# hungdinhxuan/real-time-deepfake-speech-detection

Hardware: AMD Instinct MI355X
Metric: utterances/sec (4 s @ 16 kHz) (higher is better)
Workload: dtype fp16

## Files before the change

real-time-deepfake-speech-detection_amd/csrc/afx_conformer.hip:

```cpp
#include "afx_common.h"
#include "afx_kernels.h"

namespace afx {

__global__ void conf_tokens_kernel(const float* __restrict__ ll, const float* __restrict__ cls, float bn_scale,
                                   float bn_shift, int T, int E, float* __restrict__ out, int raw) {
  const int b = blockIdx.y;
  const long n = (long)(T + 1) * E;
  for (long i = (long)blockIdx.x * blockDim.x + threadIdx.x; i < n; i += (long)gridDim.x * blockDim.x) {
    const int row = (int)(i / E), c = (int)(i % E);
    float v;
    if (row == 0)
      v = cls[c];
    else if (raw)
      v = ll[((long)b * T + row - 1) * E + c];
    else
      v = selu(fmaf(ll[((long)b * T + row - 1) * E + c], bn_scale, bn_shift));
    out[(long)b * n + i] = v;
  }
}
const char* launch_conf_tokens(const float* ll, const float* cls, float bn_scale, float bn_shift, int B, int T,
                               int E, float* out, hipStream_t s, bool raw) {
  hipLaunchKernelGGL(conf_tokens_kernel, dim3(16, B), dim3(256), 0, s, ll, cls, bn_scale, bn_shift, T, E, out, raw ? 1 : 0);
  hipError_t e = hipGetLastError();
  return e == hipSuccess ? nullptr : hipGetErrorString(e);
}

template <int DH, class HT, bool REL>
__global__ __launch_bounds__(256) void conf_attn_kernel(const float* __restrict__ q, long ldq,
                                                        const float* __restrict__ kv, long ldkv,
                                                        const float* __restrict__ rel, int max_pos, int N, int H,
                                                        int KB, typename HT::T* __restrict__ out, long ldo,
                                                        const int* __restrict__ lens, int len_add) {
  typedef typename HT::T Tt;
  extern __shared__ __attribute__((aligned(16))) float sm_f[];
  const int Nrow = N;
  if (lens) N = lens[blockIdx.y] + len_add;

  const int i0 = blockIdx.z * 256;
  const int nq = min(256, N - i0);
  float* Ks = sm_f;
  float* Vs = Ks + (long)KB * DH;
  float* Es = Vs + (long)KB * DH;
  const int h = blockIdx.x, b = blockIdx.y, tid = threadIdx.x;
  const int inner = H * DH;
  const bool live = tid < nq;
  const int i = i0 + (live ? tid : nq - 1);
  const float scale = 1.0f / sqrtf((float)DH);
  float qv[DH], o[DH];
  const float* qrow = q + ((long)b * Nrow + i) * ldq + h * DH;
#pragma unroll
  for (int d = 0; d < DH; d += 4) {
    const f32x4 t = *(const f32x4*)(qrow + d);
    qv[d] = t[0] * scale; qv[d + 1] = t[1] * scale; qv[d + 2] = t[2] * scale; qv[d + 3] = t[3] * scale;
    o[d] = o[d + 1] = o[d + 2] = o[d + 3] = 0.f;
  }
  float m = -1e30f, l = 0.f;
  for (int jb = 0; jb < N; jb += KB) {
    const int nk = min(KB, N - jb);
    if (jb) __syncthreads();
    for (int idx = tid; idx < nk * (DH / 4); idx += 256) {
// ... 60 lines not shown
  Tt* orow = out + ((long)b * Nrow + i) * ldo + h * DH;
#pragma unroll
  for (int d = 0; d < DH; d += 4) {
    typename HT::V4 v4;
    v4[0] = (Tt)(o[d] * rl); v4[1] = (Tt)(o[d + 1] * rl); v4[2] = (Tt)(o[d + 2] * rl); v4[3] = (Tt)(o[d + 3] * rl);
    *(typename HT::V4*)(orow + d) = v4;
  }
}

static int g_conf_attn_block = 0;
void conf_attn_set_block(int v) { g_conf_attn_block = v > 0 ? (v + 3) & ~3 : 0; }

template <int DH, class HT, bool REL>
static hipError_t launch_conf_attn_t(const float* q, long ldq, const float* kv, long ldkv, const float* rel,
                                     int max_pos, int B, int N, int H, void* out, long ldo, hipStream_t s,
                                     const int* lens, int len_add) {
  auto lds_of = [&](int kb) { return (int)((2L * kb + (REL ? min(256, N) + kb - 1 : 0)) * DH * sizeof(float)); };
  int KB = N;
  if (g_conf_attn_block && g_conf_attn_block < N) KB = g_conf_attn_block;
  else if (N > 256 || lds_of(N) > 160 * 1024) KB = 64;
  const int lds = lds_of(KB);
  static LdsLimit lim;
  if (hipError_t e = lim.ensure((const void*)conf_attn_kernel<DH, HT, REL>, lds); e != hipSuccess) return e;
  hipLaunchKernelGGL((conf_attn_kernel<DH, HT, REL>), dim3(H, B, (N + 255) / 256), dim3(256), lds, s, q, ldq, kv, ldkv, rel,
                     max_pos, N, H, KB, (typename HT::T*)out, ldo, lens, len_add);
  return hipGetLastError();
}

const char* launch_conf_attn(const float* q, long ldq, const float* kv, long ldkv, const float* rel, int max_pos,
                             int B, int N, int H, int dh, void* out_h, long ldo, int dtype, hipStream_t s,
                             const int* lens, int len_add) {
  if (N <= 0 || B <= 0 || B > 65535) return "conf_attn: bad shape";
  if ((ldq % 4) || (ldkv % 4) || (ldo % 4)) return "conf_attn: row strides must be multiples of 4";
  hipError_t e = hipSuccess;
#define AFX_CA(DHv)                                                                                             \
  AFX_DISPATCH_HT(dtype, e = launch_conf_attn_t<DHv, HT, true>(q, ldq, kv, ldkv, rel, max_pos, B, N, H, out_h, ldo, s, lens, len_add))
  if (!rel) {
    if (dh != 64 || dtype != DT_FP32) return "conf_attn: the no-relative-term form is the fp32 trunk attention (dh 64)";
    e = launch_conf_attn_t<64, F32T, false>(q, ldq, kv, ldkv, nullptr, 0, B, N, H, out_h, ldo, s, lens, len_add);
  }
  else if (dh == 36) { AFX_CA(36); }
  else if (dh == 32) { AFX_CA(32); }
  else if (dh == 64) { AFX_CA(64); }
  else return "conf_attn: supported head dims are 32, 36 (emb 144 / 4 heads) and 64";
#undef AFX_CA
  return e == hipSuccess ? nullptr : hipGetErrorString(e);
}

constexpr int CA_KEYS = 224, CA_VT_STRIDE = 232, CA_RS = 228, CA_NKT = 14, CA_KS = 7;

template <class HT, int DH, int NW>
__global__ __launch_bounds__(64 * NW) void conf_attn_mfma_kernel(const float* __restrict__ q, long ldq,
                                                             const float* __restrict__ kv, long ldkv,
                                                             const typename HT::T* __restrict__ rel_h, int max_pos,
                                                             int N, int H, typename HT::T* __restrict__ out, long ldo,
                                                             const int* __restrict__ lens, int len_add) {
  typedef typename HT::T Tt;
  typedef typename HT::V8 V8;
  typedef typename HT::V4 V4;
  const int Nrow = N;
  if (lens) N = lens[blockIdx.y] + len_add;
  constexpr int DT = (DH + 15) / 16;
  static_assert(DH % 4 == 0 && DH <= 64, "head dim");
  extern __shared__ __attribute__((aligned(16))) float sm_f[];
  char* sm = (char*)sm_f;
  char* k_lds = sm;
  Tt* vt_lds = (Tt*)(sm + CA_KEYS * 128);
  float* r_lds = (float*)(sm + CA_KEYS * 128 + 16 * DT * CA_VT_STRIDE * 2);
  constexpr int NT = 64 * NW;

  const int h = blockIdx.x, b = blockIdx.y;
// ... 22 lines not shown
        V4 kh;
#pragma unroll
        for (int i = 0; i < 4; ++i) kh[i] = (Tt)kreg[it][i];
        const int c = q4 >> 1;
        *(V4*)(k_lds + key * 128 + ((c ^ ((key >> 1) & 7)) * 16) + (q4 & 1) * 8) = kh;
#pragma unroll
        for (int i = 0; i < 4; ++i) vt_lds[(q4 * 4 + i) * CA_VT_STRIDE + key] = (Tt)vreg[it][i];
      }
    }
  }
  __syncthreads();

  const int ql = lane & 15, g = lane >> 4;
  const float scale = 1.0f / sqrtf((float)DH);
  float* rw = r_lds + wave * 16 * CA_RS;
  const int nqt = (N + 15) >> 4;
  for (int qt = wave; qt < nqt; qt += NW) {
    const int q0 = qt * 16;
    int qrow = q0 + ql;
    qrow = qrow < N ? qrow : N - 1;
    V8 qf[2];
    {
      const float* qp = q + ((long)b * Nrow + qrow) * ldq + h * DH;
#pragma unroll
      for (int ks = 0; ks < 2; ++ks)
#pragma unroll
        for (int half = 0; half < 2; ++half) {
          const int d = ks * 32 + g * 8 + half * 4;
          f32x4 t = f32x4{0.f, 0.f, 0.f, 0.f};
          if (d < DH) t = *(const f32x4*)(qp + d);
#pragma unroll
// ... 118 lines not shown
        const int d = nt * 16 + g * 4;
        if (d < DH) {
          V4 hv;
#pragma unroll
          for (int c = 0; c < 4; ++c) hv[c] = (Tt)(o[nt][c] * rinv);
          *(V4*)(out + ((long)b * Nrow + qi) * ldo + h * DH + d) = hv;
        }
      }
    }
  }
}

template <int DH, int NW>
__global__ __launch_bounds__(64 * NW) void conf_attn_split_kernel(const float* __restrict__ q, long ldq, const float* __restrict__ kv, long ldkv,
                                                                  const float* __restrict__ rel64, int max_pos, int N, int H,
                                                                  float* __restrict__ out, long ldo, const int* __restrict__ lens, int len_add) {
  typedef _Float16 Tt;
  typedef f16x8 V8;
  typedef f16x4 V4;
  const int Nrow = N;
  if (lens) N = lens[blockIdx.y] + len_add;
  constexpr int DT = (DH + 15) / 16;
  static_assert(DH % 4 == 0 && DH <= 64, "head dim");
  extern __shared__ __attribute__((aligned(16))) float sm_f[];
  char* sm = (char*)sm_f;
  constexpr int KB = CA_KEYS * 128, VB = 16 * DT * CA_VT_STRIDE * 2;
  char* k_lds[2] = {sm, sm + KB};
  Tt* vt_lds[2] = {(Tt*)(sm + 2 * KB), (Tt*)(sm + 2 * KB + VB)};
  float* r_lds = (float*)(sm + 2 * KB + 2 * VB);
  constexpr int NT = 64 * NW;
  const int h = blockIdx.x, b = blockIdx.y;
// ... 43 lines not shown
        *(V4*)(k_lds[0] + off) = kh;
        *(V4*)(k_lds[1] + off) = kl;
#pragma unroll
        for (int i = 0; i < 4; ++i) {
          vt_lds[0][(q4 * 4 + i) * CA_VT_STRIDE + key] = vh[i];
          vt_lds[1][(q4 * 4 + i) * CA_VT_STRIDE + key] = vl[i];
        }
      }
    }
  }
  __syncthreads();

  const int ql = lane & 15, g = lane >> 4;
  const float scale = 1.0f / sqrtf((float)DH);
  float* rw = r_lds + wave * 16 * CA_RS;
  const int nqt = (N + 15) >> 4;
  for (int qt = wave; qt < nqt; qt += NW) {
    const int q0 = qt * 16;
    int qrow = q0 + ql;
    qrow = qrow < N ? qrow : N - 1;
    V8 qh[2], qlo[2];
    {
      const float* qp = q + ((long)b * Nrow + qrow) * ldq + h * DH;
#pragma unroll
      for (int ks = 0; ks < 2; ++ks) {
        f32x4 t[2];
#pragma unroll
        for (int half = 0; half < 2; ++half) {
          const int d = ks * 32 + g * 8 + half * 4;
          t[half] = f32x4{0.f, 0.f, 0.f, 0.f};
          if (d < DH) t[half] = *(const f32x4*)(qp + d);
// ... 129 lines not shown
#pragma unroll
      for (int nt = 0; nt < DT; ++nt) {
        const int d = nt * 16 + g * 4;
        if (d < DH) *(f32x4*)(out + ((long)b * Nrow + qi) * ldo + h * DH + d) = o[nt] * rinv;
      }
#ifdef SHAW_DBG
      if (g == 0) {
        out[((long)b * Nrow + qi) * ldo + h * DH + 0] = mx;
        out[((long)b * Nrow + qi) * ldo + h * DH + 1] = sum;
      }
#endif
    }
  }
}
const char* launch_conf_attn_split(const float* q, long ldq, const float* kv, long ldkv, const float* rel64, int max_pos, int B, int N,
                                   int H, int dh, float* out, long ldo, hipStream_t s, const int* lens, int len_add) {
  if (dh != 36) return "conf_attn_split: built for head dim 36 (emb 144 / 4 heads)";
  if (N <= 0 || N + 15 > CA_KEYS || B <= 0 || B > 65535) return "conf_attn_split: 1..209 tokens";
  if ((ldq % 4) || (ldkv % 4) || (ldo % 4)) return "conf_attn_split: row strides must be multiples of 4";
  constexpr int DT = 3, NW = 4;
  const int lds = 2 * CA_KEYS * 128 + 2 * 16 * DT * CA_VT_STRIDE * 2 + NW * 16 * CA_RS * 4;
  static LdsLimit lim;
  hipError_t e = lim.ensure((const void*)conf_attn_split_kernel<36, NW>, lds);
  if (e == hipSuccess) {
    hipLaunchKernelGGL((conf_attn_split_kernel<36, NW>), dim3(H, B), dim3(64 * NW), lds, s, q, ldq, kv, ldkv, rel64, max_pos, N, H, out, ldo, lens, len_add);
    e = hipGetLastError();
  }
  return e == hipSuccess ? nullptr : hipGetErrorString(e);
}

constexpr int CAL_KB = 128, CAL_VT_STRIDE = 136, CAL_RS = 148, CAL_NKT = 8, CAL_KS = 4, CAL_RT = 9;

template <class HT, int DH>
__global__ __launch_bounds__(256, 2) void conf_attn_mfma_long_kernel(const float* __restrict__ q, long ldq,
                                                                  const float* __restrict__ kv, long ldkv,
                                                                  const typename HT::T* __restrict__ rel_h, int max_pos,
                                                                  int N, int H, typename HT::T* __restrict__ out, long ldo,
                                                                  const int* __restrict__ lens, int len_add) {
  typedef typename HT::T Tt;
  typedef typename HT::V8 V8;
// ... 159 lines not shown
#pragma unroll
        for (int c = 0; c < 4; ++c) hv[c] = (Tt)(o[nt][c] * rinv);
        *(V4*)(out + ((long)b * Nrow + qi) * ldo + h * DH + d) = hv;
      }
    }
  }
}

static int g_conf_attn_force_long = 0;
void conf_attn_mfma_set_force_long(int v) { g_conf_attn_force_long = v != 0; }
static int g_conf_attn_waves = 7;
void conf_attn_mfma_set_waves(int v) { g_conf_attn_waves = v == 4 ? 4 : 7; }

const char* launch_conf_attn_mfma(const float* q, long ldq, const float* kv, long ldkv, const void* rel_h, int max_pos,
                                  int B, int N, int H, int dh, void* out_h, long ldo, int dtype, hipStream_t s,
                                  const int* lens, int len_add) {
  if (dh != 36) return "conf_attn_mfma: built for head dim 36 (emb 144 / 4 heads)";
  if (N <= 0 || B <= 0 || B > 65535) return "conf_attn_mfma: bad shape";
  if (dtype == DT_FP32) return "conf_attn_mfma: half-precision operands only";
  if ((ldq % 4) || (ldkv % 4) || (ldo % 4)) return "conf_attn_mfma: row strides must be multiples of 4";
  constexpr int DT = 3;
  if (N + 15 > CA_KEYS || g_conf_attn_force_long) {
    const int ldsl = CAL_KB * 128 + 16 * DT * CAL_VT_STRIDE * 2 + 4 * 16 * CAL_RS * 4;
    hipError_t el = hipSuccess;
    static LdsLimit liml[2];
    dim3 grid(H, B, (N + 63) / 64);
    if (dtype == DT_BF16) {
      el = liml[0].ensure((const void*)conf_attn_mfma_long_kernel<BF16, 36>, ldsl);
      if (el == hipSuccess)
        hipLaunchKernelGGL((conf_attn_mfma_long_kernel<BF16, 36>), grid, dim3(256), ldsl, s, q, ldq, kv, ldkv, (const __bf16*)rel_h,
                           max_pos, N, H, (__bf16*)out_h, ldo, lens, len_add);
    } else {
      el = liml[1].ensure((const void*)conf_attn_mfma_long_kernel<FP16, 36>, ldsl);
      if (el == hipSuccess)
        hipLaunchKernelGGL((conf_attn_mfma_long_kernel<FP16, 36>), grid, dim3(256), ldsl, s, q, ldq, kv, ldkv, (const _Float16*)rel_h,
                           max_pos, N, H, (_Float16*)out_h, ldo, lens, len_add);
    }
    if (el == hipSuccess) el = hipGetLastError();
    return el == hipSuccess ? nullptr : hipGetErrorString(el);
  }
  const int nw = N > 64 && g_conf_attn_waves != 4 ? 7 : 4;
  const int lds = CA_KEYS * 128 + 16 * DT * CA_VT_STRIDE * 2 + nw * 16 * CA_RS * 4;
  hipError_t e = hipSuccess;
  static LdsLimit lim[4];
#define AFX_CAM(HTv, NWv, slot, Tv)                                                                                      \
  do {                                                                                                                   \
    e = lim[slot].ensure((const void*)conf_attn_mfma_kernel<HTv, 36, NWv>, lds);                                         \
    if (e == hipSuccess)                                                                                                 \
      hipLaunchKernelGGL((conf_attn_mfma_kernel<HTv, 36, NWv>), dim3(H, B), dim3(64 * NWv), lds, s, q, ldq, kv, ldkv,    \
                         (const Tv*)rel_h, max_pos, N, H, (Tv*)out_h, ldo, lens, len_add);                               \
  } while (0)
  if (dtype == DT_BF16) {
    if (nw == 7) AFX_CAM(BF16, 7, 0, __bf16); else AFX_CAM(BF16, 4, 1, __bf16);
  } else {
    if (nw == 7) AFX_CAM(FP16, 7, 2, _Float16); else AFX_CAM(FP16, 4, 3, _Float16);
  }
#undef AFX_CAM
  if (e == hipSuccess) e = hipGetLastError();
  return e == hipSuccess ? nullptr : hipGetErrorString(e);
}

template <class HT>
__global__ __launch_bounds__(256) void conf_dwconv_kernel(const float* __restrict__ x, long ldx,
                                                          const float* __restrict__ w, const float* __restrict__ bias,
                                                          const float* __restrict__ bn_scale,
                                                          const float* __restrict__ bn_shift, int N, int NC, int C, int k,
                                                          typename HT::T* __restrict__ out, long ldo,
                                                          const int* __restrict__ lens, int len_add) {
  typedef typename HT::T Tt;
  const int Nrow = N;
  if (lens) N = lens[blockIdx.y] + len_add;
  constexpr bool EXACT = sizeof(Tt) == 4;
  constexpr int KMAX = 31, TB = 8;
  extern __shared__ __attribute__((aligned(16))) float sm_f[];
  float* sm = sm_f;
  const int c0 = blockIdx.x * 32, b = blockIdx.y, tid = threadIdx.x;
  const int pl = k / 2;
  const int f0 = blockIdx.z * NC, nc = min(NC, N - f0);
  const int rows = nc + KMAX - 1 + TB;
  float* us = sm;
  const int cl = tid & 31, tl = tid >> 5;
  const int c = c0 + cl;
  const bool cok = c < C;
  for (int r = tl; r < rows; r += 8) {
    const int t = f0 + r - pl;
    float u = 0.f;
    if (cok && t >= 0 && t < N) {
      const float* row = x + ((long)b * Nrow + t) * ldx;
      u = row[c] * (EXACT ? sigmoid_acc(row[C + c]) : sigmoid_fast(row[C + c]));
    }
    us[r * 32 + cl] = u;
  }
  float wr[KMAX];
#pragma unroll
  for (int j = 0; j < KMAX; ++j) wr[j] = (cok && j < k) ? w[(long)c * k + j] : 0.f;
  const float bi = cok ? bias[c] : 0.f, sc = cok ? bn_scale[c] : 0.f, sh = cok ? bn_shift[c] : 0.f;
  __syncthreads();
  const int per = (nc + 7) / 8;
  const int t_end = min(nc, (tl + 1) * per);
  for (int t0 = tl * per; t0 < t_end; t0 += TB) {
    float win[TB + KMAX - 1];
#pragma unroll
// ... 5 lines not shown
    for (int j = 0; j < KMAX; ++j)
#pragma unroll
      for (int u = 0; u < TB; ++u) acc[u] = fmaf(wr[j], win[u + j], acc[u]);
    if (cok) {
#pragma unroll
      for (int u = 0; u < TB; ++u) {
        const float y = fmaf(acc[u], sc, sh);
        if (t0 + u < t_end) out[((long)b * Nrow + f0 + t0 + u) * ldo + c] = (Tt)(EXACT ? swish(y) : swish_fast(y));
      }
    }
  }
}

const char* launch_conf_dwconv(const float* x, long ldx, const float* w, const float* bias, const float* bn_scale,
                               const float* bn_shift, int B, int N, int C, int k, void* out_h, long ldo, int dtype,
                               hipStream_t s, const int* lens, int len_add) {
  if (k > 31) return "conf_dwconv: depthwise kernels up to 31 taps";
  if (N <= 0 || B <= 0 || B > 65535) return "conf_dwconv: bad shape";
  const int NC = N < 1024 ? N : 1024;
  const int lds = (NC + 31 - 1 + 8) * 32 * (int)sizeof(float);
  dim3 grid((C + 31) / 32, B, (N + NC - 1) / NC);
  hipError_t e = hipSuccess;
  static LdsLimit lim[3];
  if (dtype < 0 || dtype > 2) return "conf_dwconv: unknown dtype";
  AFX_DISPATCH_HT(dtype, {
    e = lim[dtype].ensure((const void*)conf_dwconv_kernel<HT>, lds);
    if (e == hipSuccess)
      hipLaunchKernelGGL(conf_dwconv_kernel<HT>, grid, dim3(256), lds, s, x, ldx, w, bias, bn_scale, bn_shift, N, NC, C, k,
                         (HT::T*)out_h, ldo, lens, len_add);
  });
  if (e == hipSuccess) e = hipGetLastError();
  return e == hipSuccess ? nullptr : hipGetErrorString(e);
}

__global__ void small_linear_kernel(const float* __restrict__ x, long row_stride, int rows, int K,
                                    const float* __restrict__ w, const float* __restrict__ b, int N,
                                    float* __restrict__ out, int* __restrict__ nonfinite) {
  const int lane = threadIdx.x & 63;
  const int r = blockIdx.x * (blockDim.x >> 6) + (threadIdx.x >> 6);
  if (r >= rows) return;
  const float* xr = x + (long)r * row_stride;
  for (int n = 0; n < N; ++n) {
    float a = 0.f;
    for (int kk = lane; kk < K; kk += 64) a = fmaf(xr[kk], w[(long)n * K + kk], a);
// ... 18 lines not shown
```

real-time-deepfake-speech-detection_amd/csrc/afx_conformer_fused.hip:

```cpp
#include "afx_common.h"
#include "afx_kernels.h"

#ifndef CHAIN_DBG
#define CHAIN_DBG 0
#endif

namespace afx {

namespace {

constexpr int ET = 9;
constexpr int EK = 5;
constexpr int HT6 = 6;
constexpr int RING = 4, BUFSZ = 32 * 1024, DUMP = RING * BUFSZ;
constexpr int PARAMS = DUMP + 1024;
#ifndef CHAIN_NWAVE
#define CHAIN_NWAVE 4
#endif
constexpr int NWAVE = CHAIN_NWAVE;
constexpr int DPW = 32 / NWAVE;
static_assert(NWAVE == 8 || NWAVE == 4, "wave count");
template <int N>
__device__ __forceinline__ void chain_wait_vmcnt() {
  static_assert(N >= 0 && N < 64, "vmcnt is a 6-bit counter");
// ... 299 lines not shown
    for (int j = 0; j < ET; ++j) {
      const f32x4 bb = *(const f32x4*)(prm + CP_FF_B2 + j * 16 + kq * 4);
      x[j] += 0.5f * (o[j] + bb);
    }
  }
};

}

template <class HT, int STAGE, bool S3>
__global__ __launch_bounds__(64 * NWAVE) void conf_chain_kernel(ConfChainArgs p) {
  typedef Chain<HT, STAGE, S3> C;
  typedef typename C::AF AF;
  extern __shared__ __attribute__((aligned(16))) char smem[];
  C c(p, smem);
  const long row = ((long)blockIdx.x * NWAVE + c.wave) * 16 + c.r16;
  const bool ok = row < p.M;
  const long rc = ok ? row : p.M - 1;

  f32x4 x[ET];
#pragma unroll
  for (int j = 0; j < ET; ++j) x[j] = *(const f32x4*)(p.x_in + rc * p.E + j * 16 + c.kq * 4);
  AF ain[ET];
  if constexpr (STAGE != 0) {
#pragma unroll
    for (int t = 0; t < (STAGE == 1 ? EK : ET); ++t) ain[t] = c.load_frag(p.in_h, rc, p.ld_in_h, t * 32 + c.kb);
  }
#pragma unroll
  for (int j = 0; j < ET; ++j) asm volatile("" : "+v"(x[j]));
  if constexpr (STAGE != 0) {
#pragma unroll
    for (int t = 0; t < (STAGE == 1 ? EK : ET); ++t) {
      asm volatile("" : "+v"(ain[t].h));
// ... 66 lines not shown
    c.feed_forward(x);
    f32x4 y[ET];
    c.layernorm(x, c.prm + CP_LN2_G, c.prm + CP_LN2_B, y);
    if (ok) {
#pragma unroll
      for (int j = 0; j < ET; ++j) *(f32x4*)(p.x_out + row * p.E + j * 16 + c.kq * 4) = y[j];
    }
  }
}

template <class HT, int STAGE, bool S3>
static hipError_t launch_conf_chain_t(const ConfChainArgs& p, hipStream_t s) {
  constexpr int lds = PARAMS + (kChainParamFloats + (S3 ? kChainScaleFloats : 0)) * 4;
  static LdsLimit lim;
  if (hipError_t e = lim.ensure((const void*)conf_chain_kernel<HT, STAGE, S3>, lds); e != hipSuccess) return e;
  hipLaunchKernelGGL((conf_chain_kernel<HT, STAGE, S3>), dim3((unsigned)((p.M + 16 * NWAVE - 1) / (16 * NWAVE))), dim3(64 * NWAVE), lds, s, p);
  return hipGetLastError();
}

const char* launch_conf_chain(const ConfChainArgs& p, int stage, int dtype, hipStream_t s) {
  if (p.E != 16 * ET || p.Ep < 32 * EK || p.FFp != 4 * 16 * ET) return "conf_chain: the fused Conformer chains are built for emb 144 / ff 576";
  if (dtype == DT_FP32) return "conf_chain: half-precision operands only";
  if (p.M <= 0 || stage < 0 || stage > 2) return "conf_chain: bad arguments";
  hipError_t e;
  if (dtype == DT_FP16X3)
    e = stage == 0 ? launch_conf_chain_t<FP16, 0, true>(p, s) : stage == 1 ? launch_conf_chain_t<FP16, 1, true>(p, s) : launch_conf_chain_t<FP16, 2, true>(p, s);
  else if (dtype == DT_BF16)
    e = stage == 0 ? launch_conf_chain_t<BF16, 0, false>(p, s) : stage == 1 ? launch_conf_chain_t<BF16, 1, false>(p, s) : launch_conf_chain_t<BF16, 2, false>(p, s);
  else
    e = stage == 0 ? launch_conf_chain_t<FP16, 0, false>(p, s) : stage == 1 ? launch_conf_chain_t<FP16, 1, false>(p, s) : launch_conf_chain_t<FP16, 2, false>(p, s);
  return e == hipSuccess ? nullptr : hipGetErrorString(e);
}

}
```

real-time-deepfake-speech-detection_amd/csrc/afx_engine.hip:

```cpp
#include <hip/hip_runtime.h>

#include <algorithm>
#include <cmath>
#include <cstdarg>
#include <cstdio>
#include <cstring>
#include <string>
#include <unordered_map>
#include <unordered_set>
#include <vector>

#include "../../include/afx.h"
#include "afx_common.h"
#include "afx_kernels.h"
#include "afx_aasist.h"

using namespace afx;

static thread_local char g_err[512] = "";
static int fail(const char* fmt, ...) {
  va_list ap;
  va_start(ap, fmt);
  vsnprintf(g_err, sizeof g_err, fmt, ap);
  va_end(ap);
// ... 590 lines not shown
    off += bytes;
    return p;
  }
};

struct Ws {
  int T[7];
  void *bufA = nullptr, *bufB = nullptr, *feats_h = nullptr, *xpad = nullptr, *hbuf = nullptr, *qkv = nullptr, *att = nullptr, *ff = nullptr,
       *ssl_h = nullptr;
  float *tmp32 = nullptr, *x = nullptr, *ssl_f = nullptr;
  void* s3planes = nullptr;
  size_t s3bytes = 0;
  float* gn_stats = nullptr;
  int* lens = nullptr;
  float *bucket_f = nullptr, *bucket_logits = nullptr;
  float *ll32 = nullptr, *xc = nullptr, *qkv32 = nullptr, *glu32 = nullptr;
  void *hc = nullptr, *hid = nullptr, *ao = nullptr, *u = nullptr;
  AasistWs aa;
};

static size_t carve(const afx_engine* e, int B, int L, int Tfeat, void* base, Ws* w, int T5 = 0, bool ragged = false) {
  Carver c(base);
  const size_t hs = dtype_size(e->dt);
  int T = Tfeat;
  w->lens = nullptr;
  w->bucket_f = w->bucket_logits = nullptr;
  if (L > 0 || T5 > 0) {
    if (L > 0) {
      conv_lengths(L, w->T);
      const size_t n0 = (size_t)B * w->T[0] * kC, n1 = (size_t)B * w->T[1] * kC;
// ... 462 lines not shown
    n2.out_h = w.hbuf; n2.ldo_h = kD;
    KOK(launch_rownorm(n2, dt, s));
    TAP(lp + "ln2", w.hbuf, (size_t)M * kD, true, kD);
    GemmArgs f1 = plain_gemm(w.hbuf, kD, e->w1[l], kD, M, kF, kD);
    f1.bias = e->F(P + "fc1.bias"); f1.act = ACT_GELU;
    f1.out_h = w.ff; f1.ldo_h = kF;
    KOK(launch_gemm(f1, dt, 1, s));
    TAP(lp + "ff", w.ff, (size_t)M * kF, true, kF);
    KOK(resid_product(w.ff, kF, e->w2[l], kF, e->F(P + "fc2.bias")));
    if (e->taps_on) {
      const std::string nm = "layer" + std::to_string(l);
      if (tap(e, nm.c_str(), w.x, (size_t)M * kD, false, s)) return 1;
    }
  }
  RowNormArgs nf = plain_norm(w.x, kD, M, kD, e->F("ssl.encoder.layer_norm.weight"), e->F("ssl.encoder.layer_norm.bias"));
  nf.out_f = w.ssl_f; nf.ldo_f = kD;
  nf.out_h = w.ssl_h; nf.ldo_h = kD;
  nf.nonfinite = e->nonfinite;
  KOK(launch_rownorm(nf, dt, s));
  if (tap(e, "ssl", w.ssl_f, (size_t)M * kD, false, s)) return 1;
  return 0;
}

static int run_conformer(afx_engine* e, int B, int T, Ws& w, float* logits, hipStream_t s, const float* tokens = nullptr,
                         float* embedding = nullptr) {
  const int dt = e->dt, E = e->E, Ep = e->Ep, N = T + 1, M = B * N;
  if (tokens) {
    KOK(timed(PC_MISC, 0, s, [&] { return launch_conf_tokens(tokens, e->F("conformer.class_token"), 1.f, 0.f, B, T, E, w.xc, s, true); }));
  } else {
    GemmArgs ll = plain_gemm(w.ssl_h, kD, e->conf_ll, kD, B * T, E, kD);
    ll.bias = e->F("LL.bias");
// ... 9 lines not shown
  const int chain_dt = e->s3 ? DT_FP16X3 : dt;
  HIP_OK(hipMemsetAsync(w.ao, 0, (size_t)M * Ep * hs, s));
  if (!fused) {
    HIP_OK(hipMemsetAsync(w.hc, 0, (size_t)M * Ep * hs, s));
    HIP_OK(hipMemsetAsync(w.u, 0, (size_t)M * e->C2p * hs, s));
    if (e->FFp != e->FF) HIP_OK(hipMemsetAsync(w.hid, 0, (size_t)M * e->FFp * hs, s));
  }
  for (int b = 0; fused && b < e->nblk; ++b) {
    const std::string P = "conformer.encoder_blocks." + std::to_string(b) + ".";
    ConfBlock& K = e->blk[b];
    ConfChainArgs c;
    memset(&c, 0, sizeof c);
    c.M = M; c.E = E; c.Ep = Ep; c.FFp = e->FFp;
    c.x_in = w.xc; c.x_out = w.xc;
    auto ff = [&](void* w1, void* w2) { c.ff_w1 = w1; c.ff_w2 = w2; };
    const double ff_fl = 2.0 * M * E * e->FF * 2;
    ff(K.ff1_w1, K.ff1_w2);
    c.params = K.chain_prm[0];
    c.w_a = K.wqkv; c.ld_w_a = Ep;
    c.out2 = w.qkv32; c.ld_out2 = 3 * e->inner;
    KOK(timed(PC_CONF_CHAIN, ff_fl + 2.0 * M * E * 3 * e->inner, s, [&] { return launch_conf_chain(c, 0, chain_dt, s); }));
    const std::string bp = "b" + std::to_string(b) + ".";
    TAP(bp + "xa", w.xc, (size_t)M * E, false, E);
    TAP(bp + "qkv", w.qkv32, (size_t)M * 3 * e->inner, false, 3 * e->inner);
    KOK(timed(PC_CONF_ATTN, 6.0 * B * e->heads * (double)N * N * e->dh, s, [&] {
      if (e->conf_attn_mfma && dt != DT_FP32 && e->dh == 36)
        return launch_conf_attn_mfma(w.qkv32, 3 * e->inner, w.qkv32 + e->inner, 3 * e->inner, K.rel_h, 512, B, N, e->heads,
                                     e->dh, w.ao, Ep, dt, s, w.lens, 1);
      if (e->conf_attn_mfma && e->s3 && e->dh == 36 && N <= 209)
        return launch_conf_attn_split(w.qkv32, 3 * e->inner, w.qkv32 + e->inner, 3 * e->inner, (const float*)K.rel_h, 512, B, N,
                                      e->heads, e->dh, (float*)w.ao, Ep, s, w.lens, 1);
      return launch_conf_attn(w.qkv32, 3 * e->inner, w.qkv32 + e->inner, 3 * e->inner,
                              e->F(P + "attn.fn.rel_pos_emb.weight"), 512, B, N, e->heads, e->dh, w.ao, Ep, dt, s, w.lens, 1);
    }));
    TAP(bp + "ao", w.ao, (size_t)M * Ep, true, Ep);
    c.in_h = w.ao; c.ld_in_h = Ep;
    c.params = K.chain_prm[1];
    c.w_a = K.wout;
    c.w_b = K.pw1;
    c.out2 = w.glu32; c.ld_out2 = 2 * e->C2;
    KOK(timed(PC_CONF_CHAIN, 2.0 * M * E * (e->inner + 2 * e->C2), s, [&] { return launch_conf_chain(c, 1, chain_dt, s); }));
    TAP(bp + "xb", w.xc, (size_t)M * E, false, E);
    TAP(bp + "glu", w.glu32, (size_t)M * 2 * e->C2, false, 2 * e->C2);
    KOK(timed(PC_CONF_DWCONV, 2.0 * B * N * e->C2 * e->ck, s, [&] {
      return launch_conf_dwconv(w.glu32, 2 * e->C2, e->F(P + "conv.net.4.conv.weight"),
                                e->F(P + "conv.net.4.conv.bias"), K.bn_scale, K.bn_shift, B, N, e->C2, e->ck, w.u,
                                e->C2p, dt, s, w.lens, 1);
    }));
    TAP(bp + "u", w.u, (size_t)M * e->C2p, true, e->C2p);
    c.in_h = w.u; c.ld_in_h = e->C2p;
    c.params = K.chain_prm[2];
    c.w_a = K.pw2; c.ld_w_a = e->C2p;
    ff(K.ff2_w1, K.ff2_w2);
    c.w_b = nullptr; c.out2 = nullptr;
    KOK(timed(PC_CONF_CHAIN, ff_fl + 2.0 * M * e->C2 * E, s, [&] { return launch_conf_chain(c, 2, chain_dt, s); }));
    if (e->taps_on) {
      const std::string nm = "block" + std::to_string(b);
      if (tap(e, nm.c_str(), w.xc, (size_t)M * E, false, s)) return 1;
    }
  }
  for (int b = 0; !fused && b < e->nblk; ++b) {
    const std::string P = "conformer.encoder_blocks." + std::to_string(b) + ".";
    ConfBlock& K = e->blk[b];
    const std::string bp = "b" + std::to_string(b) + ".";
    auto norm_to_h = [&](const char* nm) -> const char* {
      RowNormArgs n = plain_norm(w.xc, E, M, E, e->F(P + nm + ".weight"), e->F(P + nm + ".bias"));
      n.out_h = w.hc; n.ldo_h = Ep;
      return launch_rownorm(n, dt, s);
    };
    auto feed_forward = [&](const char* ff, void* w1, void* w2) -> int {
// ... 1101 lines not shown
    for (int k = 0; k < nb; ++k)
      HIP_OK(hipMemcpyAsync(logits + (size_t)idx[k] * 2, w.bucket_logits + (size_t)k * 2, 8, hipMemcpyDeviceToDevice, s));
  }
  return 0;
}

extern "C" int afx_ssl_forward_ragged(afx_handle h, const float* wave, int B, int Lmax, const int* n_samples, float* feats,
                                      int* n_frames, void* ws, size_t ws_bytes, void* stream) {
  if (check_call(h, wave, B, Lmax, feats, ws, true)) return 1;
  if (!n_samples) return fail("afx_ssl_forward_ragged: null lengths");
  if (h->cfg.pre_emphasis) return fail("afx_ssl_forward_ragged: engine-side pre-emphasis is not supported on ragged batches");
  if (h->cfg.extractor_mode == AFX_EXTRACTOR_GROUP_NORM) return fail("afx_ssl_forward_ragged: the group-norm extractor normalises over the whole clip; zero padding would enter its statistics");
  Ws w;
  const size_t needb = carve(h, B, Lmax, 0, ws, &w, 0, true);
  if (ws_bytes < needb) return fail("afx_ssl_forward_ragged: workspace too small (%zu < %zu bytes)", ws_bytes, needb);
  hipStream_t s = (hipStream_t)stream;
  std::vector<int> frames;
  if (ragged_setup(h, B, Lmax, n_samples, w, frames, s)) return 1;
  begin_call(h, &w);
  if (run_trunk(h, wave, B, Lmax, w, s)) return 1;
  const int Tmax = w.T[6];
  HIP_OK(hipMemcpyAsync(feats, w.ssl_f, (size_t)B * Tmax * kD * 4, hipMemcpyDeviceToDevice, s));
  for (int b = 0; b < B; ++b) {
    if (frames[b] < Tmax)
      HIP_OK(hipMemsetAsync(feats + ((size_t)b * Tmax + frames[b]) * kD, 0, (size_t)(Tmax - frames[b]) * kD * 4, s));
    if (n_frames) n_frames[b] = frames[b];
  }
  return 0;
}

extern "C" int afx_ssl_forward(afx_handle h, const float* wave, int B, int L, float* feats, void* ws, size_t ws_bytes,
                               void* stream) {
  if (check_call(h, wave, B, L, feats, ws, true)) return 1;
  Ws w;
  const size_t needb = carve(h, B, L, 0, ws, &w);
  if (ws_bytes < needb) return fail("afx_ssl_forward: workspace too small (%zu < %zu bytes)", ws_bytes, needb);
  hipStream_t s = (hipStream_t)stream;
  begin_call(h, &w);
  if (run_trunk(h, wave, B, L, w, s)) return 1;
  HIP_OK(hipMemcpyAsync(feats, w.ssl_f, (size_t)B * w.T[6] * kD * 4, hipMemcpyDeviceToDevice, s));
  return 0;
}

__global__ void f32_to_half_kernel(const float* in, uint16_t* out, size_t n, int is_bf16) {
  for (size_t i = (size_t)blockIdx.x * blockDim.x + threadIdx.x; i < n; i += (size_t)gridDim.x * blockDim.x) {
    if (is_bf16) {
      __bf16 v = (__bf16)in[i];
      memcpy(&out[i], &v, 2);
    } else {
      _Float16 v = (_Float16)in[i];
      memcpy(&out[i], &v, 2);
// ... 287 lines not shown
```

real-time-deepfake-speech-detection_amd/csrc/afx_kernels.h:

```cpp
#pragma once
#include <hip/hip_runtime.h>
#include <stdint.h>

namespace afx {

enum DType { DT_BF16 = 0, DT_FP16 = 1, DT_FP32 = 2, DT_FP16X3 = 3 };
inline size_t dtype_size(int dt) { return dt == DT_FP32 || dt == DT_FP16X3 ? 4 : 2; }
constexpr float kS3ScaleBounded = 16.f;
constexpr float kS3ScaleFree = 1.f;
__host__ __device__ inline long s3_pair_index(long k) { return ((k >> 5) << 6) + (k & 31); }

struct GemmArgs {
  const void* A;
  const void* W;
  int M, N, K;
  int k_algo;
  int rpb;
  long a_batch, a_row;
  int kchunk;
  long kchunk_stride;
  long ldw;
  long g_a, g_w;
  int g_n;
  const float* bias;
// ... 114 lines not shown
                              bool out_pairs = false, float out_scale = 1.f);
const char* launch_mhsa_ring(const void* ring, void* out, int S, int H, int q_tile, const int* cnt, int dtype, hipStream_t s);
const char* launch_mhsa_ring_split(const float* ring, float* out, int S, int H, int q_tile, const int* cnt, hipStream_t s,
                                   bool out_pairs = false, float out_scale = 1.f);
const char* launch_mhsa_ring_tab(const void* ring, void* out, int S, int H, int q_tile, const int* tab, int dtype, hipStream_t s);
const char* launch_mhsa_ring_split_tab(const float* ring, float* out, int S, int H, int q_tile, const int* tab, hipStream_t s,
                                       bool out_pairs, float out_scale);
const char* launch_mhsa_ring_active(const void* ring, void* out, int A, int H, const int* tab, int dtype, hipStream_t s);
const char* launch_mhsa_ring_split_active(const float* ring, float* out, int A, int H, const int* tab, hipStream_t s, bool out_pairs,
                                          float out_scale);

const char* launch_conf_tokens(const float* ll, const float* cls, float bn_scale, float bn_shift, int B, int T,
                               int E, float* out, hipStream_t s, bool raw = false);
const char* launch_conf_attn(const float* q, long ldq, const float* kv, long ldkv, const float* rel, int max_pos,
                             int B, int N, int H, int dh, void* out_h, long ldo, int dtype, hipStream_t s,
                             const int* lens = nullptr, int len_add = 0);
const char* launch_conf_attn_split(const float* q, long ldq, const float* kv, long ldkv, const float* rel64, int max_pos, int B, int N,
                                   int H, int dh, float* out, long ldo, hipStream_t s, const int* lens = nullptr, int len_add = 0);
const char* launch_conf_attn_mfma(const float* q, long ldq, const float* kv, long ldkv, const void* rel_h, int max_pos,
                                  int B, int N, int H, int dh, void* out_h, long ldo, int dtype, hipStream_t s,
                                  const int* lens = nullptr, int len_add = 0);
const char* launch_conf_dwconv(const float* x, long ldx, const float* w , const float* bias,
                               const float* bn_scale, const float* bn_shift, int B, int N, int C, int k,
                               void* out_h, long ldo, int dtype, hipStream_t s, const int* lens = nullptr, int len_add = 0);
enum ChainParamOffsets { CP_FF_G = 0, CP_FF_B = 144, CP_FF_B1 = 288, CP_FF_B2 = 864, CP_LN2_G = 1008, CP_LN2_B = 1152,
                         CP_BA = 1296, CP_BB = 1440 };
constexpr int kChainParamFloats = 2048;
constexpr int kChainScaleFloats = 2048;
enum ChainScaleOffsets { CS_FF1 = 0, CS_FF2 = 576, CS_A = 720, CS_B = 1152 };
static_assert(CS_B + 576 <= kChainScaleFloats, "scale block");
struct ConfChainArgs {
  int M, E, Ep, FFp;
  const float* x_in;
  float* x_out;
  const float* params;
  const void *ff_w1, *ff_w2;
  const void* w_a;
  int ld_w_a;
  const void* w_b;
  const void* in_h;
  long ld_in_h;
  float* out2;
  long ld_out2;
};
const char* launch_conf_chain(const ConfChainArgs& p, int stage, int dtype, hipStream_t s);
const char* launch_small_linear(const float* x, long row_stride, int rows, int K, const float* w, const float* b,
                                int N, float* out, hipStream_t s, int* nonfinite = nullptr);

}
```

Measured before the change: 13650.

## Trim last conformer block to the rows that feed the CLS output

In the final conformer block, when taps are off, attention computes only the first query tile, the conv chain processes only the rows inside the depthwise conv's receptive field of the CLS token, and the final FF chain processes only the CLS row per utterance. The row-tiling parameters are threaded through the attention, dwconv and fused chain kernels. Separately, the fp32 SSL feature output of the trunk layer norm is skipped for the conformer path unless it is requested. This removes work whose results are never read, at the cost of leaving the other rows of the last block stale in the workspace.

```diff
diff --git a/real-time-deepfake-speech-detection_amd/csrc/afx_conformer.hip b/real-time-deepfake-speech-detection_amd/csrc/afx_conformer.hip
--- a/real-time-deepfake-speech-detection_amd/csrc/afx_conformer.hip
+++ b/real-time-deepfake-speech-detection_amd/csrc/afx_conformer.hip
@@ -31,7 +31,7 @@
                                                         const float* __restrict__ kv, long ldkv,
                                                         const float* __restrict__ rel, int max_pos, int N, int H,
                                                         int KB, typename HT::T* __restrict__ out, long ldo,
-                                                        const int* __restrict__ lens, int len_add) {
+                                                        const int* __restrict__ lens, int len_add, int q_rows) {
   typedef typename HT::T Tt;
   extern __shared__ __attribute__((aligned(16))) float sm_f[];
   const int Nrow = N;
@@ -44,7 +44,7 @@
   float* Es = Vs + (long)KB * DH;
   const int h = blockIdx.x, b = blockIdx.y, tid = threadIdx.x;
   const int inner = H * DH;
-  const bool live = tid < nq;
+  const bool live = tid < nq && i0 + tid < q_rows;
   const int i = i0 + (live ? tid : nq - 1);
   const float scale = 1.0f / sqrtf((float)DH);
   float qv[DH], o[DH];
@@ -135,7 +135,7 @@
 template <int DH, class HT, bool REL>
 static hipError_t launch_conf_attn_t(const float* q, long ldq, const float* kv, long ldkv, const float* rel,
                                      int max_pos, int B, int N, int H, void* out, long ldo, hipStream_t s,
-                                     const int* lens, int len_add) {
+                                     const int* lens, int len_add, int q_tiles) {
   auto lds_of = [&](int kb) { return (int)((2L * kb + (REL ? min(256, N) + kb - 1 : 0)) * DH * sizeof(float)); };
   int KB = N;
   if (g_conf_attn_block && g_conf_attn_block < N) KB = g_conf_attn_block;
@@ -143,22 +143,23 @@
   const int lds = lds_of(KB);
   static LdsLimit lim;
   if (hipError_t e = lim.ensure((const void*)conf_attn_kernel<DH, HT, REL>, lds); e != hipSuccess) return e;
-  hipLaunchKernelGGL((conf_attn_kernel<DH, HT, REL>), dim3(H, B, (N + 255) / 256), dim3(256), lds, s, q, ldq, kv, ldkv, rel,
-                     max_pos, N, H, KB, (typename HT::T*)out, ldo, lens, len_add);
+  const int q_rows = q_tiles > 0 && q_tiles * 16 < N ? q_tiles * 16 : N;
+  hipLaunchKernelGGL((conf_attn_kernel<DH, HT, REL>), dim3(H, B, (q_rows + 255) / 256), dim3(256), lds, s, q, ldq, kv, ldkv, rel,
+                     max_pos, N, H, KB, (typename HT::T*)out, ldo, lens, len_add, q_rows);
   return hipGetLastError();
 }
 
 const char* launch_conf_attn(const float* q, long ldq, const float* kv, long ldkv, const float* rel, int max_pos,
                              int B, int N, int H, int dh, void* out_h, long ldo, int dtype, hipStream_t s,
-                             const int* lens, int len_add) {
+                             const int* lens, int len_add, int q_tiles) {
   if (N <= 0 || B <= 0 || B > 65535) return "conf_attn: bad shape";
   if ((ldq % 4) || (ldkv % 4) || (ldo % 4)) return "conf_attn: row strides must be multiples of 4";
   hipError_t e = hipSuccess;
 #define AFX_CA(DHv)                                                                                             \
-  AFX_DISPATCH_HT(dtype, e = launch_conf_attn_t<DHv, HT, true>(q, ldq, kv, ldkv, rel, max_pos, B, N, H, out_h, ldo, s, lens, len_add))
+  AFX_DISPATCH_HT(dtype, e = launch_conf_attn_t<DHv, HT, true>(q, ldq, kv, ldkv, rel, max_pos, B, N, H, out_h, ldo, s, lens, len_add, q_tiles))
   if (!rel) {
     if (dh != 64 || dtype != DT_FP32) return "conf_attn: the no-relative-term form is the fp32 trunk attention (dh 64)";
-    e = launch_conf_attn_t<64, F32T, false>(q, ldq, kv, ldkv, nullptr, 0, B, N, H, out_h, ldo, s, lens, len_add);
+    e = launch_conf_attn_t<64, F32T, false>(q, ldq, kv, ldkv, nullptr, 0, B, N, H, out_h, ldo, s, lens, len_add, q_tiles);
   }
   else if (dh == 36) { AFX_CA(36); }
   else if (dh == 32) { AFX_CA(32); }
@@ -175,7 +176,7 @@
                                                              const float* __restrict__ kv, long ldkv,
                                                              const typename HT::T* __restrict__ rel_h, int max_pos,
                                                              int N, int H, typename HT::T* __restrict__ out, long ldo,
-                                                             const int* __restrict__ lens, int len_add) {
+                                                             const int* __restrict__ lens, int len_add, int q_tiles) {
   typedef typename HT::T Tt;
   typedef typename HT::V8 V8;
   typedef typename HT::V4 V4;
@@ -228,7 +229,7 @@
   const int ql = lane & 15, g = lane >> 4;
   const float scale = 1.0f / sqrtf((float)DH);
   float* rw = r_lds + wave * 16 * CA_RS;
-  const int nqt = (N + 15) >> 4;
+  const int nqt = min((N + 15) >> 4, q_tiles);
   for (int qt = wave; qt < nqt; qt += NW) {
     const int q0 = qt * 16;
     int qrow = q0 + ql;
@@ -377,7 +378,8 @@
 template <int DH, int NW>
 __global__ __launch_bounds__(64 * NW) void conf_attn_split_kernel(const float* __restrict__ q, long ldq, const float* __restrict__ kv, long ldkv,
                                                                   const float* __restrict__ rel64, int max_pos, int N, int H,
-                                                                  float* __restrict__ out, long ldo, const int* __restrict__ lens, int len_add) {
+                                                                  float* __restrict__ out, long ldo, const int* __restrict__ lens, int len_add,
+                                                                  int q_tiles) {
   typedef _Float16 Tt;
   typedef f16x8 V8;
   typedef f16x4 V4;
@@ -451,7 +453,7 @@
   const int ql = lane & 15, g = lane >> 4;
   const float scale = 1.0f / sqrtf((float)DH);
   float* rw = r_lds + wave * 16 * CA_RS;
-  const int nqt = (N + 15) >> 4;
+  const int nqt = min((N + 15) >> 4, q_tiles);
   for (int qt = wave; qt < nqt; qt += NW) {
     const int q0 = qt * 16;
     int qrow = q0 + ql;
@@ -611,7 +613,7 @@
   }
 }
 const char* launch_conf_attn_split(const float* q, long ldq, const float* kv, long ldkv, const float* rel64, int max_pos, int B, int N,
-                                   int H, int dh, float* out, long ldo, hipStream_t s, const int* lens, int len_add) {
+                                   int H, int dh, float* out, long ldo, hipStream_t s, const int* lens, int len_add, int q_tiles) {
   if (dh != 36) return "conf_attn_split: built for head dim 36 (emb 144 / 4 heads)";
   if (N <= 0 || N + 15 > CA_KEYS || B <= 0 || B > 65535) return "conf_attn_split: 1..209 tokens";
   if ((ldq % 4) || (ldkv % 4) || (ldo % 4)) return "conf_attn_split: row strides must be multiples of 4";
@@ -620,7 +622,8 @@
   static LdsLimit lim;
   hipError_t e = lim.ensure((const void*)conf_attn_split_kernel<36, NW>, lds);
   if (e == hipSuccess) {
-    hipLaunchKernelGGL((conf_attn_split_kernel<36, NW>), dim3(H, B), dim3(64 * NW), lds, s, q, ldq, kv, ldkv, rel64, max_pos, N, H, out, ldo, lens, len_add);
+    hipLaunchKernelGGL((conf_attn_split_kernel<36, NW>), dim3(H, B), dim3(64 * NW), lds, s, q, ldq, kv, ldkv, rel64, max_pos, N, H, out, ldo, lens, len_add,
+                       q_tiles > 0 ? q_tiles : CA_NKT);
     e = hipGetLastError();
   }
   return e == hipSuccess ? nullptr : hipGetErrorString(e);
@@ -810,7 +813,7 @@
 
 const char* launch_conf_attn_mfma(const float* q, long ldq, const float* kv, long ldkv, const void* rel_h, int max_pos,
                                   int B, int N, int H, int dh, void* out_h, long ldo, int dtype, hipStream_t s,
-                                  const int* lens, int len_add) {
+                                  const int* lens, int len_add, int q_tiles) {
   if (dh != 36) return "conf_attn_mfma: built for head dim 36 (emb 144 / 4 heads)";
   if (N <= 0 || B <= 0 || B > 65535) return "conf_attn_mfma: bad shape";
   if (dtype == DT_FP32) return "conf_attn_mfma: half-precision operands only";
@@ -835,6 +838,7 @@
     if (el == hipSuccess) el = hipGetLastError();
     return el == hipSuccess ? nullptr : hipGetErrorString(el);
   }
+  const int nqt = q_tiles > 0 ? q_tiles : CA_NKT;
   const int nw = N > 64 && g_conf_attn_waves != 4 ? 7 : 4;
   const int lds = CA_KEYS * 128 + 16 * DT * CA_VT_STRIDE * 2 + nw * 16 * CA_RS * 4;
   hipError_t e = hipSuccess;
@@ -844,7 +848,7 @@
     e = lim[slot].ensure((const void*)conf_attn_mfma_kernel<HTv, 36, NWv>, lds);                                         \
     if (e == hipSuccess)                                                                                                 \
       hipLaunchKernelGGL((conf_attn_mfma_kernel<HTv, 36, NWv>), dim3(H, B), dim3(64 * NWv), lds, s, q, ldq, kv, ldkv,    \
-                         (const Tv*)rel_h, max_pos, N, H, (Tv*)out_h, ldo, lens, len_add);                               \
+                         (const Tv*)rel_h, max_pos, N, H, (Tv*)out_h, ldo, lens, len_add, nqt);                          \
   } while (0)
   if (dtype == DT_BF16) {
     if (nw == 7) AFX_CAM(BF16, 7, 0, __bf16); else AFX_CAM(BF16, 4, 1, __bf16);
@@ -862,7 +866,7 @@
                                                           const float* __restrict__ bn_scale,
                                                           const float* __restrict__ bn_shift, int N, int NC, int C, int k,
                                                           typename HT::T* __restrict__ out, long ldo,
-                                                          const int* __restrict__ lens, int len_add) {
+                                                          const int* __restrict__ lens, int len_add, int out_tokens) {
   typedef typename HT::T Tt;
   const int Nrow = N;
   if (lens) N = lens[blockIdx.y] + len_add;
@@ -872,8 +876,9 @@
   float* sm = sm_f;
   const int c0 = blockIdx.x * 32, b = blockIdx.y, tid = threadIdx.x;
   const int pl = k / 2;
-  const int f0 = blockIdx.z * NC, nc = min(NC, N - f0);
+  const int f0 = blockIdx.z * NC, nc = min(NC, min(N, out_tokens) - f0);
   const int rows = nc + KMAX - 1 + TB;
+  const int t_in = min(N, f0 + nc + k - 1 - pl);
   float* us = sm;
   const int cl = tid & 31, tl = tid >> 5;
   const int c = c0 + cl;
@@ -881,7 +886,7 @@
   for (int r = tl; r < rows; r += 8) {
     const int t = f0 + r - pl;
     float u = 0.f;
-    if (cok && t >= 0 && t < N) {
+    if (cok && t >= 0 && t < t_in) {
       const float* row = x + ((long)b * Nrow + t) * ldx;
       u = row[c] * (EXACT ? sigmoid_acc(row[C + c]) : sigmoid_fast(row[C + c]));
     }
@@ -917,12 +922,13 @@
 
 const char* launch_conf_dwconv(const float* x, long ldx, const float* w, const float* bias, const float* bn_scale,
                                const float* bn_shift, int B, int N, int C, int k, void* out_h, long ldo, int dtype,
-                               hipStream_t s, const int* lens, int len_add) {
+                               hipStream_t s, const int* lens, int len_add, int out_tokens) {
   if (k > 31) return "conf_dwconv: depthwise kernels up to 31 taps";
   if (N <= 0 || B <= 0 || B > 65535) return "conf_dwconv: bad shape";
-  const int NC = N < 1024 ? N : 1024;
+  if (out_tokens <= 0 || out_tokens > N) out_tokens = N;
+  const int NC = out_tokens < 1024 ? out_tokens : 1024;
   const int lds = (NC + 31 - 1 + 8) * 32 * (int)sizeof(float);
-  dim3 grid((C + 31) / 32, B, (N + NC - 1) / NC);
+  dim3 grid((C + 31) / 32, B, (out_tokens + NC - 1) / NC);
   hipError_t e = hipSuccess;
   static LdsLimit lim[3];
   if (dtype < 0 || dtype > 2) return "conf_dwconv: unknown dtype";
@@ -930,7 +936,7 @@
     e = lim[dtype].ensure((const void*)conf_dwconv_kernel<HT>, lds);
     if (e == hipSuccess)
       hipLaunchKernelGGL(conf_dwconv_kernel<HT>, grid, dim3(256), lds, s, x, ldx, w, bias, bn_scale, bn_shift, N, NC, C, k,
-                         (HT::T*)out_h, ldo, lens, len_add);
+                         (HT::T*)out_h, ldo, lens, len_add, out_tokens);
   });
   if (e == hipSuccess) e = hipGetLastError();
   return e == hipSuccess ? nullptr : hipGetErrorString(e);
diff --git a/real-time-deepfake-speech-detection_amd/csrc/afx_conformer_fused.hip b/real-time-deepfake-speech-detection_amd/csrc/afx_conformer_fused.hip
--- a/real-time-deepfake-speech-detection_amd/csrc/afx_conformer_fused.hip
+++ b/real-time-deepfake-speech-detection_amd/csrc/afx_conformer_fused.hip
@@ -337,9 +337,10 @@
   typedef typename C::AF AF;
   extern __shared__ __attribute__((aligned(16))) char smem[];
   C c(p, smem);
-  const long row = ((long)blockIdx.x * NWAVE + c.wave) * 16 + c.r16;
-  const bool ok = row < p.M;
-  const long rc = ok ? row : p.M - 1;
+  const long tile = (long)blockIdx.x * NWAVE + c.wave;
+  const long row0 = tile * p.tile_stride, row = row0 + c.r16;
+  const bool ok = tile < p.tiles && c.r16 < p.tile_rows && row < p.M;
+  const long rc = ok ? row : (tile < p.tiles ? row0 : p.M - 1);
 
   f32x4 x[ET];
 #pragma unroll
@@ -436,14 +437,22 @@
   constexpr int lds = PARAMS + (kChainParamFloats + (S3 ? kChainScaleFloats : 0)) * 4;
   static LdsLimit lim;
   if (hipError_t e = lim.ensure((const void*)conf_chain_kernel<HT, STAGE, S3>, lds); e != hipSuccess) return e;
-  hipLaunchKernelGGL((conf_chain_kernel<HT, STAGE, S3>), dim3((unsigned)((p.M + 16 * NWAVE - 1) / (16 * NWAVE))), dim3(64 * NWAVE), lds, s, p);
+  hipLaunchKernelGGL((conf_chain_kernel<HT, STAGE, S3>), dim3((unsigned)((p.tiles + NWAVE - 1) / NWAVE)), dim3(64 * NWAVE), lds, s, p);
   return hipGetLastError();
 }
 
-const char* launch_conf_chain(const ConfChainArgs& p, int stage, int dtype, hipStream_t s) {
+const char* launch_conf_chain(const ConfChainArgs& args, int stage, int dtype, hipStream_t s) {
+  ConfChainArgs p = args;
+  if (p.M <= 0 || stage < 0 || stage > 2) return "conf_chain: bad arguments";
+  if (!p.tile_stride && !p.tile_rows && !p.tiles) {
+    p.tile_stride = p.tile_rows = 16;
+    p.tiles = (p.M + 15) / 16;
+  }
+  if (p.tile_rows < 1 || p.tile_rows > 16 || p.tile_stride < p.tile_rows || p.tiles < 1 ||
+      (long)(p.tiles - 1) * p.tile_stride >= p.M)
+    return "conf_chain: bad row tiles (1..16 rows per tile, tiles must not overlap, every tile starts inside the M rows)";
   if (p.E != 16 * ET || p.Ep < 32 * EK || p.FFp != 4 * 16 * ET) return "conf_chain: the fused Conformer chains are built for emb 144 / ff 576";
   if (dtype == DT_FP32) return "conf_chain: half-precision operands only";
-  if (p.M <= 0 || stage < 0 || stage > 2) return "conf_chain: bad arguments";
   hipError_t e;
   if (dtype == DT_FP16X3)
     e = stage == 0 ? launch_conf_chain_t<FP16, 0, true>(p, s) : stage == 1 ? launch_conf_chain_t<FP16, 1, true>(p, s) : launch_conf_chain_t<FP16, 2, true>(p, s);
diff --git a/real-time-deepfake-speech-detection_amd/csrc/afx_engine.hip b/real-time-deepfake-speech-detection_amd/csrc/afx_engine.hip
--- a/real-time-deepfake-speech-detection_amd/csrc/afx_engine.hip
+++ b/real-time-deepfake-speech-detection_amd/csrc/afx_engine.hip
@@ -628,6 +628,7 @@
   float* gn_stats = nullptr;
   int* lens = nullptr;
   float *bucket_f = nullptr, *bucket_logits = nullptr;
+  bool want_ssl_f = false;
   float *ll32 = nullptr, *xc = nullptr, *qkv32 = nullptr, *glu32 = nullptr;
   void *hc = nullptr, *hid = nullptr, *ao = nullptr, *u = nullptr;
   AasistWs aa;
@@ -1120,7 +1121,9 @@
     }
   }
   RowNormArgs nf = plain_norm(w.x, kD, M, kD, e->F("ssl.encoder.layer_norm.weight"), e->F("ssl.encoder.layer_norm.bias"));
-  nf.out_f = w.ssl_f; nf.ldo_f = kD;
+  if (e->cfg.arch != AFX_ARCH_CONFORMER || w.want_ssl_f || e->taps_on) {
+    nf.out_f = w.ssl_f; nf.ldo_f = kD;
+  }
   nf.out_h = w.ssl_h; nf.ldo_h = kD;
   nf.nonfinite = e->nonfinite;
   KOK(launch_rownorm(nf, dt, s));
@@ -1160,24 +1163,28 @@
     c.M = M; c.E = E; c.Ep = Ep; c.FFp = e->FFp;
     c.x_in = w.xc; c.x_out = w.xc;
     auto ff = [&](void* w1, void* w2) { c.ff_w1 = w1; c.ff_w2 = w2; };
-    const double ff_fl = 2.0 * M * E * e->FF * 2;
+    const int conv_rows = std::min(N, e->ck - e->ck / 2);
+    const bool trim = b == e->nblk - 1 && !e->taps_on && conv_rows <= 16;
+    const int rows_b = trim ? B * conv_rows : M, rows_c = trim ? B : M;
+    auto ff_fl = [&](double rows) { return 2.0 * rows * E * e->FF * 2; };
     ff(K.ff1_w1, K.ff1_w2);
     c.params = K.chain_prm[0];
     c.w_a = K.wqkv; c.ld_w_a = Ep;
     c.out2 = w.qkv32; c.ld_out2 = 3 * e->inner;
-    KOK(timed(PC_CONF_CHAIN, ff_fl + 2.0 * M * E * 3 * e->inner, s, [&] { return launch_conf_chain(c, 0, chain_dt, s); }));
+    KOK(timed(PC_CONF_CHAIN, ff_fl(M) + 2.0 * M * E * 3 * e->inner, s, [&] { return launch_conf_chain(c, 0, chain_dt, s); }));
     const std::string bp = "b" + std::to_string(b) + ".";
     TAP(bp + "xa", w.xc, (size_t)M * E, false, E);
     TAP(bp + "qkv", w.qkv32, (size_t)M * 3 * e->inner, false, 3 * e->inner);
-    KOK(timed(PC_CONF_ATTN, 6.0 * B * e->heads * (double)N * N * e->dh, s, [&] {
+    const int q_tiles = trim ? 1 : 0;
+    KOK(timed(PC_CONF_ATTN, 6.0 * B * e->heads * (double)(trim ? std::min(N, 16) : N) * N * e->dh, s, [&] {
       if (e->conf_attn_mfma && dt != DT_FP32 && e->dh == 36)
         return launch_conf_attn_mfma(w.qkv32, 3 * e->inner, w.qkv32 + e->inner, 3 * e->inner, K.rel_h, 512, B, N, e->heads,
-                                     e->dh, w.ao, Ep, dt, s, w.lens, 1);
+                                     e->dh, w.ao, Ep, dt, s, w.lens, 1, q_tiles);
       if (e->conf_attn_mfma && e->s3 && e->dh == 36 && N <= 209)
         return launch_conf_attn_split(w.qkv32, 3 * e->inner, w.qkv32 + e->inner, 3 * e->inner, (const float*)K.rel_h, 512, B, N,
-                                      e->heads, e->dh, (float*)w.ao, Ep, s, w.lens, 1);
+                                      e->heads, e->dh, (float*)w.ao, Ep, s, w.lens, 1, q_tiles);
       return launch_conf_attn(w.qkv32, 3 * e->inner, w.qkv32 + e->inner, 3 * e->inner,
-                              e->F(P + "attn.fn.rel_pos_emb.weight"), 512, B, N, e->heads, e->dh, w.ao, Ep, dt, s, w.lens, 1);
+                              e->F(P + "attn.fn.rel_pos_emb.weight"), 512, B, N, e->heads, e->dh, w.ao, Ep, dt, s, w.lens, 1, q_tiles);
     }));
     TAP(bp + "ao", w.ao, (size_t)M * Ep, true, Ep);
     c.in_h = w.ao; c.ld_in_h = Ep;
@@ -1185,13 +1192,16 @@
     c.w_a = K.wout;
     c.w_b = K.pw1;
     c.out2 = w.glu32; c.ld_out2 = 2 * e->C2;
-    KOK(timed(PC_CONF_CHAIN, 2.0 * M * E * (e->inner + 2 * e->C2), s, [&] { return launch_conf_chain(c, 1, chain_dt, s); }));
+    if (trim) {
+      c.tile_stride = N; c.tiles = B; c.tile_rows = conv_rows;
+    }
+    KOK(timed(PC_CONF_CHAIN, 2.0 * rows_b * E * (e->inner + 2 * e->C2), s, [&] { return launch_conf_chain(c, 1, chain_dt, s); }));
     TAP(bp + "xb", w.xc, (size_t)M * E, false, E);
     TAP(bp + "glu", w.glu32, (size_t)M * 2 * e->C2, false, 2 * e->C2);
-    KOK(timed(PC_CONF_DWCONV, 2.0 * B * N * e->C2 * e->ck, s, [&] {
+    KOK(timed(PC_CONF_DWCONV, 2.0 * B * (trim ? 1 : N) * e->C2 * e->ck, s, [&] {
       return launch_conf_dwconv(w.glu32, 2 * e->C2, e->F(P + "conv.net.4.conv.weight"),
                                 e->F(P + "conv.net.4.conv.bias"), K.bn_scale, K.bn_shift, B, N, e->C2, e->ck, w.u,
-                                e->C2p, dt, s, w.lens, 1);
+                                e->C2p, dt, s, w.lens, 1, trim ? 1 : 0);
     }));
     TAP(bp + "u", w.u, (size_t)M * e->C2p, true, e->C2p);
     c.in_h = w.u; c.ld_in_h = e->C2p;
@@ -1199,7 +1209,8 @@
     c.w_a = K.pw2; c.ld_w_a = e->C2p;
     ff(K.ff2_w1, K.ff2_w2);
     c.w_b = nullptr; c.out2 = nullptr;
-    KOK(timed(PC_CONF_CHAIN, ff_fl + 2.0 * M * e->C2 * E, s, [&] { return launch_conf_chain(c, 2, chain_dt, s); }));
+    if (trim) c.tile_rows = 1;
+    KOK(timed(PC_CONF_CHAIN, ff_fl(rows_c) + 2.0 * rows_c * e->C2 * E, s, [&] { return launch_conf_chain(c, 2, chain_dt, s); }));
     if (e->taps_on) {
       const std::string nm = "block" + std::to_string(b);
       if (tap(e, nm.c_str(), w.xc, (size_t)M * E, false, s)) return 1;
@@ -2331,6 +2342,7 @@
   Ws w;
   const size_t needb = carve(h, B, Lmax, 0, ws, &w, 0, true);
   if (ws_bytes < needb) return fail("afx_ssl_forward_ragged: workspace too small (%zu < %zu bytes)", ws_bytes, needb);
+  w.want_ssl_f = true;
   hipStream_t s = (hipStream_t)stream;
   std::vector<int> frames;
   if (ragged_setup(h, B, Lmax, n_samples, w, frames, s)) return 1;
@@ -2352,6 +2364,7 @@
   Ws w;
   const size_t needb = carve(h, B, L, 0, ws, &w);
   if (ws_bytes < needb) return fail("afx_ssl_forward: workspace too small (%zu < %zu bytes)", ws_bytes, needb);
+  w.want_ssl_f = true;
   hipStream_t s = (hipStream_t)stream;
   begin_call(h, &w);
   if (run_trunk(h, wave, B, L, w, s)) return 1;
diff --git a/real-time-deepfake-speech-detection_amd/csrc/afx_kernels.h b/real-time-deepfake-speech-detection_amd/csrc/afx_kernels.h
--- a/real-time-deepfake-speech-detection_amd/csrc/afx_kernels.h
+++ b/real-time-deepfake-speech-detection_amd/csrc/afx_kernels.h
@@ -152,15 +152,18 @@
                                int E, float* out, hipStream_t s, bool raw = false);
 const char* launch_conf_attn(const float* q, long ldq, const float* kv, long ldkv, const float* rel, int max_pos,
                              int B, int N, int H, int dh, void* out_h, long ldo, int dtype, hipStream_t s,
-                             const int* lens = nullptr, int len_add = 0);
+                             const int* lens = nullptr, int len_add = 0,
+                             int q_tiles = 0);
 const char* launch_conf_attn_split(const float* q, long ldq, const float* kv, long ldkv, const float* rel64, int max_pos, int B, int N,
-                                   int H, int dh, float* out, long ldo, hipStream_t s, const int* lens = nullptr, int len_add = 0);
+                                   int H, int dh, float* out, long ldo, hipStream_t s, const int* lens = nullptr, int len_add = 0,
+                                   int q_tiles = 0);
 const char* launch_conf_attn_mfma(const float* q, long ldq, const float* kv, long ldkv, const void* rel_h, int max_pos,
                                   int B, int N, int H, int dh, void* out_h, long ldo, int dtype, hipStream_t s,
-                                  const int* lens = nullptr, int len_add = 0);
+                                  const int* lens = nullptr, int len_add = 0, int q_tiles = 0);
 const char* launch_conf_dwconv(const float* x, long ldx, const float* w , const float* bias,
                                const float* bn_scale, const float* bn_shift, int B, int N, int C, int k,
-                               void* out_h, long ldo, int dtype, hipStream_t s, const int* lens = nullptr, int len_add = 0);
+                               void* out_h, long ldo, int dtype, hipStream_t s, const int* lens = nullptr, int len_add = 0,
+                               int out_tokens = 0);
 enum ChainParamOffsets { CP_FF_G = 0, CP_FF_B = 144, CP_FF_B1 = 288, CP_FF_B2 = 864, CP_LN2_G = 1008, CP_LN2_B = 1152,
                          CP_BA = 1296, CP_BB = 1440 };
 constexpr int kChainParamFloats = 2048;
@@ -180,6 +183,7 @@
   long ld_in_h;
   float* out2;
   long ld_out2;
+  int tile_stride, tile_rows, tiles;
 };
 const char* launch_conf_chain(const ConfChainArgs& p, int stage, int dtype, hipStream_t s);
 const char* launch_small_linear(const float* x, long row_stride, int rows, int K, const float* w, const float* b,
```

After: 13820 (median of 4 runs). +1.3%, better.
